# rhiestan/Regard3D

Measured on NVIDIA H100. Metric: matched_image_pairs_per_sec_exhaustive, higher is better.
Workload: dtype u8

## Files before the change

regard3d_b200/csrc/k_l2_candidates.cu:

```cuda
#include "r3d_internal.cuh"
#include "tc_ptx.cuh"

namespace r3d {

using namespace tcx;

namespace {

constexpr int kMaxStages = 8;
constexpr uint32_t kTileN = 256;
constexpr uint32_t kStageBytes = 2 * kBoxBytes;
constexpr uint32_t kNormBytes = kTileN * 4;
constexpr uint32_t kConsumersF16 = kTileRows / 64;
constexpr uint32_t kConsumersU8 = kSuperRows / 64;
constexpr size_t kSmemOptIn = 232448;
static_assert(kChunk == 8, "the epilogue reduces one 8-column block of the wgmma accumulator per chunk");

__device__ __forceinline__ float quad_min4(float p0, float p1, float p2, float p3, uint32_t q) {
  const bool b1 = (q & 2u) != 0, b0 = (q & 1u) != 0;
  const float k0 = fminf(b1 ? p2 : p0, __shfl_xor_sync(0xffffffffu, b1 ? p0 : p2, 2));
  const float k1 = fminf(b1 ? p3 : p1, __shfl_xor_sync(0xffffffffu, b1 ? p1 : p3, 2));
  return fminf(b0 ? k1 : k0, __shfl_xor_sync(0xffffffffu, b0 ? k0 : k1, 1));
}

__device__ __forceinline__ int32_t min8(const int32_t (&v)[8]) {
  return __vimin3_s32(__vimin3_s32(v[0], v[1], v[2]), __vimin3_s32(v[3], v[4], v[5]), min(v[6], v[7]));
}

__device__ __forceinline__ float chunk_key(int32_t m, int32_t qn, uint32_t cid, uint32_t keep_mask) {
  return __uint_as_float((__float_as_uint((float)(m + qn)) & keep_mask) | cid);
}

__device__ __forceinline__ int32_t bracket_bound(float kmax, uint32_t keep_mask, int32_t qn) {
  const float f = __uint_as_float((__float_as_uint(kmax) & keep_mask) - keep_mask);
  return __float2int_ru(f) - 1 - qn;
}

__device__ __forceinline__ void merge_keys(float (&key)[kNumKeys], int d) {
  float y[kNumKeys];
#pragma unroll
  for (int i = 0; i < kNumKeys; ++i) y[i] = __shfl_xor_sync(0xffffffffu, key[i], d);
#pragma unroll
  for (int i = 0; i < kNumKeys; ++i) {
    float x = y[i];
#pragma unroll
    for (int j = 0; j < kNumKeys - 1; ++j) {
      const float hi = fmaxf(key[j], x);
      key[j] = fminf(key[j], x);
      x = hi;
    }
    key[kNumKeys - 1] = fminf(key[kNumKeys - 1], x);
  }
}

}

template <bool kU8, uint32_t kConsumers, uint32_t kKSteps>
__global__ void __launch_bounds__(128 * (kConsumers + 1), 1)
k_l2_candidates(const CUtensorMap* __restrict__ tmapQ, const CUtensorMap* __restrict__ tmapD,
                const PairDesc* __restrict__ pairs, const WorkItem* __restrict__ items, uint32_t n_items,
                uint32_t* __restrict__ keys_out, uint32_t nkb, uint32_t ksteps, uint32_t n_stages, uint32_t n_qbuf) {
  static_assert(kConsumers == 2 || (kU8 && kConsumers == 4), "fp16: 2 consumers; u8: 2 or 4");
  static_assert(kU8 ? (kKSteps >= 1 && kKSteps <= 8) : kKSteps == 0, "u8: 1 .. 8 k32 steps (D <= 256); fp16: 0");
  constexpr uint32_t kBoxCols = kU8 ? 128u : (uint32_t)kKBlock;
  constexpr uint32_t kQBoxes = kConsumers / 2;
  constexpr uint32_t kBlockRows = kQBoxes * kTileRows;
  constexpr uint32_t kConsumerWarps = 4 * kConsumers;
  constexpr uint32_t kProducerRegs = kConsumers == 4 ? 24u : 40u;
  constexpr uint32_t kConsumerRegs = kConsumers == 4 ? 112u : 232u;
  extern __shared__ unsigned char smem_raw[];
  const uint32_t base = (smem_u32(smem_raw) + 1023u) & ~1023u;
  const uint32_t q_base = base;
  const uint32_t q_bytes = kQBoxes * nkb * kBoxBytes;
  const uint32_t d_base = q_base + n_qbuf * q_bytes;
  const uint32_t n_base = d_base + n_stages * kStageBytes;
  const uint32_t bar_full = n_base + (kU8 ? n_stages * kNormBytes : 0u);
  const uint32_t bar_empty = bar_full + 8 * kMaxStages;
  const uint32_t bar_qfull = bar_empty + 8 * kMaxStages;
  const uint32_t bar_qempty = bar_qfull + 16;

  const uint32_t warp = threadIdx.x >> 5;
  const uint32_t lane = threadIdx.x & 31u;
  const uint32_t wg = threadIdx.x >> 7;

  if (threadIdx.x == 0) {
    for (uint32_t s = 0; s < (uint32_t)kMaxStages; ++s) {
      mbar_init(bar_full + 8 * s, 1);
      mbar_init(bar_empty + 8 * s, kConsumerWarps);
    }
    for (uint32_t qb = 0; qb < 2; ++qb) {
      mbar_init(bar_qfull + 8 * qb, 1);
      mbar_init(bar_qempty + 8 * qb, kConsumerWarps);
    }
    fence_barrier_init();
  }
  __syncthreads();

  if (wg == 0) {
    setmaxnreg_dec<kProducerRegs>();
    if (warp != 0) return;
    uint32_t stage = 0, phase = 0, qi = 0;
    for (uint32_t it = blockIdx.x; it < n_items; it += gridDim.x, ++qi) {
      const WorkItem wi = items[it];
      const PairDesc pd = pairs[wi.pair];
      const CUtensorMap* mq = tmapQ + pd.slotJ;
      const CUtensorMap* md = tmapD + pd.slotI;
      const uint32_t ntiles = pd.nI_pad / kTileN;
      const uint32_t qb = n_qbuf == 2 ? (qi & 1u) : 0u;
      const uint32_t quse = n_qbuf == 2 ? (qi >> 1) : qi;
      mbar_wait(bar_qempty + 8 * qb, (quse & 1u) ^ 1u);
      if (elect_one()) {
        mbar_arrive_expect_tx(bar_qfull + 8 * qb, q_bytes);
#pragma unroll
        for (uint32_t b = 0; b < kQBoxes; ++b)
          for (uint32_t kb = 0; kb < nkb; ++kb)
            tma_load_2d(q_base + qb * q_bytes + (b * nkb + kb) * kBoxBytes, mq, (int)(kb * kBoxCols),
                        (int)(wi.sb * kBlockRows + b * kTileRows), bar_qfull + 8 * qb);
      }
      __syncwarp();
      for (uint32_t t = 0; t < ntiles; ++t) {
        for (uint32_t kb = 0; kb < nkb; ++kb) {
          mbar_wait(bar_empty + 8 * stage, phase ^ 1u);
          if (elect_one()) {
            const uint32_t dst = d_base + stage * kStageBytes;
            const bool norms = kU8 && kb == 0;
            mbar_arrive_expect_tx(bar_full + 8 * stage, kStageBytes + (norms ? kNormBytes : 0u));
            if constexpr (kU8) {
              constexpr uint32_t kGroupsPerBox = kTileRows / kGroupRows;
              tma_load_5d(dst, md, (int)(kb * kBoxCols), 0, 0, 0, (int)(t * 2 * kGroupsPerBox), bar_full + 8 * stage);
              tma_load_5d(dst + kBoxBytes, md, (int)(kb * kBoxCols), 0, 0, 0, (int)(t * 2 * kGroupsPerBox + kGroupsPerBox),
                          bar_full + 8 * stage);
            } else {
              tma_load_2d(dst, md, (int)(kb * kBoxCols), (int)(t * kTileN), bar_full + 8 * stage);
              tma_load_2d(dst + kBoxBytes, md, (int)(kb * kBoxCols), (int)(t * kTileN + kTileRows), bar_full + 8 * stage);
            }
            if (norms) bulk_load(n_base + stage * kNormBytes, pd.normI + t * kTileN, kNormBytes, bar_full + 8 * stage);
          }
          __syncwarp();
          if (++stage == n_stages) { stage = 0; phase ^= 1u; }
        }
      }
    }
    return;
  }

  setmaxnreg_inc<kConsumerRegs>();
  const uint32_t cw = wg - 1u;
  const uint32_t q = lane & 3u;
  const uint32_t row0 = cw * 64u + (warp & 3u) * 16u + (lane >> 2);
  uint32_t stage = 0, phase = 0, qi = 0;
  for (uint32_t it = blockIdx.x; it < n_items; it += gridDim.x, ++qi) {
    const WorkItem wi = items[it];
    const PairDesc pd = pairs[wi.pair];
    const uint32_t ntiles = pd.nI_pad / kTileN;
    const uint32_t qb = n_qbuf == 2 ? (qi & 1u) : 0u;
    const uint32_t qf = (n_qbuf == 2 ? (qi >> 1) : qi) & 1u;
    const uint32_t keep_mask = ~((1u << pd.chunk_bits) - 1u);
    float key0[kNumKeys], key1[kNumKeys];
#pragma unroll
    for (int i = 0; i < kNumKeys; ++i) key0[i] = key1[i] = __uint_as_float(kKeySentinel);
    const uint32_t a_base = q_base + qb * q_bytes +
                            (kQBoxes == 1 ? cw * (kBoxBytes / 2) : (cw >> 1) * nkb * kBoxBytes + (cw & 1u) * (kBoxBytes / 2));
    if constexpr (kU8) {
      const int32_t qn0 = __ldg(pd.normJ + wi.sb * kBlockRows + row0);
      const int32_t qn1 = __ldg(pd.normJ + wi.sb * kBlockRows + row0 + 8u);
      int32_t acc[64];
      constexpr uint32_t kNkb = (kKSteps + 3) / 4;
      auto issue = [&](uint32_t h, uint32_t s0) {
        wgmma_fence();
        uint32_t s = s0;
#pragma unroll
        for (uint32_t kb = 0; kb < kNkb; ++kb) {
          const uint32_t a_lo = desc_lo(a_base + kb * kBoxBytes);
          const uint32_t b_lo = desc_lo(d_base + s * kStageBytes + h * kBoxBytes);
#pragma unroll
          for (uint32_t k = 0; k < 4 && 4 * kb + k < kKSteps; ++k)
            wgmma_m64n128k32_u8(acc, make_desc(a_lo + 2 * k), make_desc(b_lo + 2 * k), (kb | k) != 0u ? 1u : 0u);
          if (kb + 1 < kNkb && ++s == n_stages) s = 0;
        }
        wgmma_commit();
      };
      auto reduce = [&](uint32_t t, uint32_t h, uint32_t s0) {
        const int32_t* nrm = (const int32_t*)(smem_raw + (n_base + s0 * kNormBytes - smem_u32(smem_raw))) + h * 128u + 8u * q;
        const uint32_t chunk0 = t * (kTileN / kChunk) + h * (kTileN / 2 / kChunk) + q;
        const int32_t b0 = bracket_bound(key0[kNumKeys - 1], keep_mask, qn0);
        const int32_t b1 = bracket_bound(key1[kNumKeys - 1], keep_mask, qn1);
        int32_t m0[4], m1[4];
        uint32_t p0 = 0, p1 = 0;
#pragma unroll
        for (uint32_t g = 0; g < 4; ++g) {
          const int4 na = *(const int4*)(nrm + kGroupRows * g);
          const int4 nb = *(const int4*)(nrm + kGroupRows * g + 4);
          const int32_t* a = acc + 16 * g;
          const int32_t d0[8] = {na.x - 2 * a[0], na.y - 2 * a[1], na.z - 2 * a[4], na.w - 2 * a[5],
                                 nb.x - 2 * a[8], nb.y - 2 * a[9], nb.z - 2 * a[12], nb.w - 2 * a[13]};
          const int32_t d1[8] = {na.x - 2 * a[2], na.y - 2 * a[3], na.z - 2 * a[6], na.w - 2 * a[7],
                                 nb.x - 2 * a[10], nb.y - 2 * a[11], nb.z - 2 * a[14], nb.w - 2 * a[15]};
          m0[g] = min8(d0);
          m1[g] = min8(d1);
          p0 |= (m0[g] <= b0 ? 1u : 0u) << g;
          p1 |= (m1[g] <= b1 ? 1u : 0u) << g;
        }
        while (__any_sync(0xffffffffu, (p0 | p1) != 0u)) {
          int32_t y0 = 0, y1 = 0;
          uint32_t g0 = 0, g1 = 0;
#pragma unroll
          for (int g = 3; g >= 0; --g) {
            if (p0 & (1u << g)) { y0 = m0[g]; g0 = g; }
            if (p1 & (1u << g)) { y1 = m1[g]; g1 = g; }
          }
          const float x0 = p0 != 0u ? chunk_key(y0, qn0, chunk0 + 4 * g0, keep_mask) : __uint_as_float(kKeySentinel);
          const float x1 = p1 != 0u ? chunk_key(y1, qn1, chunk0 + 4 * g1, keep_mask) : __uint_as_float(kKeySentinel);
          p0 &= p0 - 1u;
          p1 &= p1 - 1u;
          key_insert_packed(x0, key0);
          key_insert_packed(x1, key1);
        }
      };
      mbar_wait(bar_qfull + 8 * qb, qf);
      for (uint32_t t = 0; t < ntiles; ++t) {
        const uint32_t s_t = stage;
#pragma unroll
        for (uint32_t kb = 0; kb < kNkb; ++kb) {
          mbar_wait(bar_full + 8 * stage, phase);
          if (++stage == n_stages) { stage = 0; phase ^= 1u; }
        }
#pragma unroll
        for (uint32_t h = 0; h < 2; ++h) {
          issue(h, s_t);
          wgmma_wait<0>();
          wgmma_fence_operand(acc);
          if (h == 1 && t + 1 == ntiles && lane == 0) mbar_arrive(bar_qempty + 8 * qb);
          reduce(t, h, s_t);
        }
        __syncwarp();
        if (lane == 0)
#pragma unroll
          for (uint32_t kb = 0, s = s_t; kb < kNkb; ++kb) {
            mbar_arrive(bar_empty + 8 * s);
            if (++s == n_stages) s = 0;
          }
      }
    } else {
      float acc[128];
      mbar_wait(bar_qfull + 8 * qb, qf);
      for (uint32_t t = 0; t < ntiles; ++t) {
        uint32_t ks_left = ksteps, prev = 0;
        for (uint32_t kb = 0; kb < nkb; ++kb) {
          mbar_wait(bar_full + 8 * stage, phase);
          wgmma_fence();
          const uint32_t a_lo = desc_lo(a_base + kb * kBoxBytes);
          const uint32_t b_lo = desc_lo(d_base + stage * kStageBytes);
          const uint32_t ks_here = ks_left < 4u ? ks_left : 4u;
#pragma unroll
          for (uint32_t k = 0; k < 4; ++k) {
            if (k < ks_here) wgmma_m64n256k16(acc, make_desc(a_lo + 2 * k), make_desc(b_lo + 2 * k), (kb | k) != 0u ? 1u : 0u);
          }
          wgmma_commit();
          if (kb > 0) {
            wgmma_wait<1>();
            if (lane == 0) mbar_arrive(bar_empty + 8 * prev);
          }
          prev = stage;
          ks_left -= ks_here;
          if (++stage == n_stages) { stage = 0; phase ^= 1u; }
        }
        wgmma_wait<0>();
        wgmma_fence_operand(acc);
        if (lane == 0) {
          mbar_arrive(bar_empty + 8 * prev);
          if (t + 1 == ntiles) mbar_arrive(bar_qempty + 8 * qb);
        }
        const uint32_t chunk0 = t * (kTileN / kChunk);
#pragma unroll
        for (uint32_t g = 0; g < 8; ++g) {
          const float* a = acc + 16 * g;
          const float m0 = quad_min4(fminf(a[0], a[1]), fminf(a[4], a[5]), fminf(a[8], a[9]), fminf(a[12], a[13]), q);
          const float m1 = quad_min4(fminf(a[2], a[3]), fminf(a[6], a[7]), fminf(a[10], a[11]), fminf(a[14], a[15]), q);
          key_insert<true>(m0, chunk0 + 4 * g + q, keep_mask, key0);
          key_insert<true>(m1, chunk0 + 4 * g + q, keep_mask, key1);
        }
      }
    }
    merge_keys(key0, 1);
    merge_keys(key0, 2);
    merge_keys(key1, 1);
    merge_keys(key1, 2);
    if (q < 2) {
      float k[kNumKeys];
#pragma unroll
      for (int i = 0; i < kNumKeys; ++i) k[i] = q == 0 ? key0[i] : key1[i];
      const uint32_t row = wi.sb * kBlockRows + row0 + 8u * q;
      uint4 o0, o1;
      o0.x = __float_as_uint(k[0]); o0.y = __float_as_uint(k[1]);
      o0.z = __float_as_uint(k[2]); o0.w = __float_as_uint(k[3]);
      o1.x = __float_as_uint(k[4]); o1.y = __float_as_uint(k[5]);
      o1.z = kKeySentinel; o1.w = kKeySentinel;
      uint4* dst = (uint4*)keys_out + (size_t)(pd.q_ofs + row) * (kKeyStride / 4);
      dst[0] = o0;
      dst[1] = o1;
    }
  }
}

static int ring_stages(uint32_t q_bytes, int n_qbuf, uint32_t stage_bytes) {
  const size_t fixed = 1024 + 8 * (2 * kMaxStages + 4) + (size_t)n_qbuf * q_bytes;
  const int stages = (int)((kSmemOptIn - fixed) / stage_bytes);
  return stages > kMaxStages ? kMaxStages : stages;
}

int launch_l2_candidates(r3d_ctx* ctx, DeviceWorker& w, const PairDesc* d_pairs, const WorkItem* d_items,
                         uint32_t n_items, uint32_t* d_keys, int dtype, uint32_t dim) {
  if (n_items == 0) return R3D_OK;
  const bool u8 = int_operand(dtype, dim);
  const int nkb = u8 ? ((int)dim + 127) / 128 : (operand_cols((int)dim) + kKBlock - 1) / kKBlock;
  const int ksteps = u8 ? ((int)dim + 31) / 32 : operand_ksteps((int)dim);
  if (nkb > kMaxKBlocks) return fail(ctx, R3D_ERR_UNSUPPORTED, "descriptor dimension too large for the tensor-core path");
  const uint32_t consumers = u8 ? kConsumersU8 : kConsumersF16;
  const uint32_t stage_bytes = kStageBytes + (u8 ? kNormBytes : 0u);
  const uint32_t q_bytes = consumers / 2 * nkb * kBoxBytes;
  const int min_stages = u8 ? 2 * nkb : 3;
  const int n_qbuf = ring_stages(q_bytes, 2, stage_bytes) >= min_stages ? 2 : 1;
  const int stages = ring_stages(q_bytes, n_qbuf, stage_bytes);
  const size_t smem = 1024 + (size_t)n_qbuf * q_bytes + (size_t)stages * stage_bytes + 8 * (2 * kMaxStages + 4);
  using Kernel = decltype(&k_l2_candidates<false, kConsumersF16, 0>);
  static const Kernel kU8Kernels[8] = {
      k_l2_candidates<true, kConsumersU8, 1>, k_l2_candidates<true, kConsumersU8, 2>, k_l2_candidates<true, kConsumersU8, 3>,
      k_l2_candidates<true, kConsumersU8, 4>, k_l2_candidates<true, kConsumersU8, 5>, k_l2_candidates<true, kConsumersU8, 6>,
      k_l2_candidates<true, kConsumersU8, 7>, k_l2_candidates<true, kConsumersU8, 8>};
  const Kernel kern = u8 ? kU8Kernels[ksteps - 1] : k_l2_candidates<false, kConsumersF16, 0>;
  R3D_CUDA_TRY(ctx, cudaFuncSetAttribute(kern, cudaFuncAttributeMaxDynamicSharedMemorySize, (int)smem));
  const uint32_t grid = n_items < (uint32_t)w.sm_count ? n_items : (uint32_t)w.sm_count;
  kern<<<grid, 128 * (consumers + 1), smem, w.stream>>>((const CUtensorMap*)w.d_tmapQ, (const CUtensorMap*)w.d_tmapD, d_pairs, d_items,
                                           n_items, d_keys, (uint32_t)nkb, (uint32_t)ksteps, (uint32_t)stages,
                                           (uint32_t)n_qbuf);
  R3D_CUDA_TRY(ctx, cudaGetLastError());
  return R3D_OK;
}

}
```

Measured before the change: 8026.

## Overlap u8 wgmma issue with key insertion of previous half-tile

New measurement: 8814 (median of 6 runs). +9.8%, better.

```diff
diff --git a/regard3d_b200/csrc/k_l2_candidates.cu b/regard3d_b200/csrc/k_l2_candidates.cu
--- a/regard3d_b200/csrc/k_l2_candidates.cu
+++ b/regard3d_b200/csrc/k_l2_candidates.cu
@@ -180,13 +180,13 @@
         }
         wgmma_commit();
       };
-      auto reduce = [&](uint32_t t, uint32_t h, uint32_t s0) {
+      int32_t m0[4], m1[4];
+      uint32_t p0, p1;
+      auto take_minima = [&](uint32_t h, uint32_t s0) {
         const int32_t* nrm = (const int32_t*)(smem_raw + (n_base + s0 * kNormBytes - smem_u32(smem_raw))) + h * 128u + 8u * q;
-        const uint32_t chunk0 = t * (kTileN / kChunk) + h * (kTileN / 2 / kChunk) + q;
         const int32_t b0 = bracket_bound(key0[kNumKeys - 1], keep_mask, qn0);
         const int32_t b1 = bracket_bound(key1[kNumKeys - 1], keep_mask, qn1);
-        int32_t m0[4], m1[4];
-        uint32_t p0 = 0, p1 = 0;
+        p0 = p1 = 0;
 #pragma unroll
         for (uint32_t g = 0; g < 4; ++g) {
           const int4 na = *(const int4*)(nrm + kGroupRows * g);
@@ -201,6 +201,9 @@
           p0 |= (m0[g] <= b0 ? 1u : 0u) << g;
           p1 |= (m1[g] <= b1 ? 1u : 0u) << g;
         }
+      };
+      auto insert = [&](uint32_t t, uint32_t h) {
+        const uint32_t chunk0 = t * (kTileN / kChunk) + h * (kTileN / 2 / kChunk) + q;
         while (__any_sync(0xffffffffu, (p0 | p1) != 0u)) {
           int32_t y0 = 0, y1 = 0;
           uint32_t g0 = 0, g1 = 0;
@@ -217,22 +220,29 @@
           key_insert_packed(x1, key1);
         }
       };
-      mbar_wait(bar_qfull + 8 * qb, qf);
-      for (uint32_t t = 0; t < ntiles; ++t) {
-        const uint32_t s_t = stage;
+      auto wait_tile = [&]() {
+        const uint32_t s0 = stage;
 #pragma unroll
         for (uint32_t kb = 0; kb < kNkb; ++kb) {
           mbar_wait(bar_full + 8 * stage, phase);
           if (++stage == n_stages) { stage = 0; phase ^= 1u; }
         }
-#pragma unroll
-        for (uint32_t h = 0; h < 2; ++h) {
-          issue(h, s_t);
-          wgmma_wait<0>();
-          wgmma_fence_operand(acc);
-          if (h == 1 && t + 1 == ntiles && lane == 0) mbar_arrive(bar_qempty + 8 * qb);
-          reduce(t, h, s_t);
-        }
+        return s0;
+      };
+      auto mma_done = [&]() {
+        wgmma_wait<0>();
+        wgmma_fence_operand(acc);
+      };
+      mbar_wait(bar_qfull + 8 * qb, qf);
+      uint32_t s_t = wait_tile();
+      issue(0, s_t);
+      mma_done();
+      take_minima(0, s_t);
+      for (uint32_t t = 0;; ++t) {
+        issue(1, s_t);
+        insert(t, 0);
+        mma_done();
+        take_minima(1, s_t);
         __syncwarp();
         if (lane == 0)
 #pragma unroll
@@ -240,6 +250,16 @@
             mbar_arrive(bar_empty + 8 * s);
             if (++s == n_stages) s = 0;
           }
+        if (t + 1 == ntiles) {
+          if (lane == 0) mbar_arrive(bar_qempty + 8 * qb);
+          insert(t, 1);
+          break;
+        }
+        s_t = wait_tile();
+        issue(0, s_t);
+        insert(t, 1);
+        mma_done();
+        take_minima(0, s_t);
       }
     } else {
       float acc[128];
```
